# yuki-koyama/sequential-line-search

Measured on AMD Instinct MI355X. Metric: GP-fit+acq-max step time (ms) and candidate-evals/sec at N=8192 D=64, higher is better.
Workload: dtype f64

## Files before the change

sequential-line-search_amd/csrc/capi.hip:

```cpp
#include <cstddef>
#include <cstring>
#include <algorithm>
#include <cmath>
#include <cstdlib>
#include <cstring>
#include <atomic>
#include <map>
#include <memory>
#include <condition_variable>
#include <mutex>
#include <shared_mutex>

#include "common.hpp"
#include "kernels.hpp"
#include "lbfgs_driver.hpp"

using namespace slsk;


namespace slsk {
static thread_local char g_err[512] = "";
void set_error(const char* fmt, ...) {
    va_list ap;
    va_start(ap, fmt);
// ... 303 lines not shown
    if (!ctx) return SLS_ERR_INVALID;
    CtxCall call_(ctx);
    (void)hipStreamSynchronize(ctx->stream);
    ctx->prof_collect();
    ctx->prof.clear();
    return SLS_OK;
}
extern "C" int sls_prof_get(sls_ctx* ctx, const char* name, double* total_ms, long* launches) {
    if (!ctx || !name) return SLS_ERR_INVALID;
    CtxCall call_(ctx);
    (void)hipStreamSynchronize(ctx->stream);
    ctx->prof_collect();
    if (std::string(name) == "potrf_fallbacks") {
        if (total_ms) *total_ms = 0.0;
        if (launches) *launches = ctx->potrf_fallbacks;
        return SLS_OK;
    }
    auto it = ctx->prof.find(name);
    if (total_ms) *total_ms = it == ctx->prof.end() ? 0.0 : it->second.ms;
    if (launches) *launches = it == ctx->prof.end() ? 0 : it->second.launches;
    return SLS_OK;
}

static void h2d(sls_ctx* c, double* dst, const double* src, size_t n) {
    SLS_HIP(hipMemcpyAsync(dst, src, n * sizeof(double), hipMemcpyHostToDevice, c->stream));
}
static void d2h(sls_ctx* c, double* dst, const double* src, size_t n) {
    SLS_HIP(hipMemcpyAsync(dst, src, n * sizeof(double), hipMemcpyDeviceToHost, c->stream));
}
static void sync(sls_ctx* c) { SLS_HIP(hipStreamSynchronize(c->stream)); }
static const size_t IO_STAGE_MAX = (size_t)4 << 20;

static void check_theta(const double* theta, int D) {
    SLS_REQUIRE(theta != nullptr, "theta is NULL");
    SLS_REQUIRE(theta[0] > 0.0, "theta[0] (signal variance) must be positive");
    for (int d = 0; d < D; ++d) SLS_REQUIRE(theta[1 + d] > 0.0, "length scale %d must be positive", d);
}

static void d2h_matrix(sls_ctx* c, double* dst, const double* src, int N, int Np) {
    SLS_HIP(hipMemcpy2DAsync(dst, (size_t)N * 8, src, (size_t)Np * 8, (size_t)N * 8, N, hipMemcpyDeviceToHost, c->stream));
}
static void h2d_matrix(sls_ctx* c, double* dst, const double* src, int N, int Np) {
    SLS_HIP(hipMemcpy2DAsync(dst, (size_t)Np * 8, src, (size_t)N * 8, (size_t)N * 8, N, hipMemcpyHostToDevice, c->stream));
}

struct sls_gp {
    sls_ctx* ctx = nullptr;
    int D = 0, N = 0, Np = 0, Dp = 0, Dcols = 0, kernel = 0;
    double a = 0, b = 0;
    std::vector<double> theta, Xh, yh;
    std::vector<double> il_h, ypad_h;
    bool host_stale = false;
    DBuf X, y, inv_ell, XT, XaT, nx, L, Linv, Kinv, U, alpha, tvec, mu_data, scal, gemv_part, idx_buf;
    const double* linv_clean_p = nullptr;
    int linv_clean_np = 0;
    long* d_idx = nullptr;
    HostBuf sum;
    int best_index = 0;
    double mu_best = 0, logdet = 0;
    DBuf Ks, Cs, P, Vs, parts, Gs, Gm, Gpart, XsT, ns, raw, outv;
    int ws_chunk = 0;
    DBuf pair_mu, pair_sg, pair_dmu, pair_dsg;
    LbfgsWs lb;
    DBuf eubo_Ks, eubo_Cs, eubo_XsT, eubo_ns, eubo_parts, eubo_Gs, eubo_Gm, eubo_Kd;
    int eubo_chunk = 0, eubo_np = 0;
    HostBuf eubo_best;
    int sigma_mode = 0;
    long generation = 0;
    long stat_issued = 0, stat_cap = 0;
    int stat_rounds = 0, stat_live_end = 0;
    HostBuf zc;
    HostBuf io;
    double* io_stage(size_t doubles) {
        if (io.host && doubles * 8 > io.bytes) (void)hipStreamSynchronize(ctx->stream);
        io.ensure(ctx, doubles * 8, false);
        return io.host;
    }
    std::shared_mutex state_mtx;
};

static bool gp_fit_small_ok(const sls_gp* g) {
    if (g->N > NLL_SMALL_MAX_N || g->Np != 128 || g->D > 128) return false;
    return tune_on(TUNE_FIT_SMALL);
}

static std::atomic<long> g_gp_generation{0};
static void gp_fit_device(sls_gp* g) {
    g->generation = ++g_gp_generation;
    sls_ctx* c = g->ctx;
    const int N = g->N, Np = g->Np, D = g->D;
    if (gp_fit_small_ok(g)) {
        GpFitSmallArgs f;
        f.X = g->X.p; f.y = g->y.p; f.inv_ell = g->inv_ell.p;
        f.D = D; f.N = N; f.Dcols = g->Dcols; f.a = g->a; f.b = g->b;
        f.XT = g->XT.p; f.nx = g->nx.p; f.XaT = g->XaT.p; f.L = g->L.p; f.Linv = g->Linv.p; f.U = g->U.p; f.Kinv = g->Kinv.p;
        f.alpha = g->alpha.p; f.mu_data = g->mu_data.p; f.scal = g->scal.p; f.d_idx = g->d_idx; f.info = c->d_info;
        f.summary = g->sum.dev;
        f.x_lds = tune_on(TUNE_SMALL_XLDS) ? 1 : 0;
        SLS_HIP(hipMemsetAsync(c->d_info, 0, 64, c->stream));
        ProfScope ps(c, "fit_small");
        launch_gp_fit_small(c->stream, g->kernel, f);
        return;
    }
    KernelSpec ks{g->kernel, g->a};
    {
        ProfScope ps(c, "gram");
        launch_prep_points(c->stream, g->X.p, D, N, g->inv_ell.p, g->XT.p, Np, Np, g->Dcols, g->nx.p);
        launch_gram_sym(c->stream, g->XT.p, Np, g->Dp, g->nx.p, Np, N, ks, g->b, g->L.p, true);
    }
    SLS_HIP(hipMemsetAsync(c->d_info, 0, 64, c->stream));
    if (g->linv_clean_p != g->Linv.p || g->linv_clean_np != Np) {
        launch_fill(c->stream, g->Linv.p, (long)Np * Np, 0.0);
        g->linv_clean_p = g->Linv.p;
        g->linv_clean_np = Np;
    }
    c->potrf_tick_rearm();
    int* df_sync = c->potrf_df_sync(Np);
    if (potri_fused_applies(Np, df_sync != nullptr)) {
        ProfScope ps(c, "potri");
        if (!launch_potri(c->stream, g->L.p, Np, g->Linv.p, g->U.p, g->Kinv.p, c->d_info, df_sync))
            ps.rename("potrf+trtri+lauum");
    } else {
        {
            ProfScope ps(c, "potrf");
            launch_potrf(c->stream, g->L.p, Np, g->Linv.p, c->d_info, 0, df_sync);
        }
        {
            ProfScope ps(c, "trtri");
            launch_trtri(c->stream, g->L.p, Np, g->Linv.p, g->Kinv.p, g->U.p);
        }
        {
            ProfScope ps(c, "lauum");
            launch_lauum(c->stream, g->U.p, Np, g->Kinv.p);
        }
    }
    launch_gemv_n(c->stream, g->Linv.p, Np, g->y.p, g->tvec.p, g->gemv_part.p, true);
    launch_gemv_t(c->stream, g->Linv.p, Np, g->tvec.p, g->alpha.p, true);
    launch_scale_rows(c->stream, g->XT.p, g->alpha.p, g->XaT.p, Np, Np, g->Dcols);
    if (g->sigma_mode == 1) launch_transpose_full(c->stream, g->Linv.p, g->U.p, Np);
    launch_fit_summary(c->stream, g->y.p, g->alpha.p, g->b, N, g->mu_data.p, g->L.p, Np, c->d_info, g->scal.p, g->d_idx, g->sum.dev);
}

static void gp_fetch_summary(sls_gp* g, int attempt = 0) {
    sls_ctx* c = g->ctx;
    sync(c);
    const double* sm = g->sum.host;
    const int info[2] = {(int)sm[3], (int)sm[4]};
    if (potrf_gave_up(c, info[1], attempt)) {
        gp_fit_device(g);
        gp_fetch_summary(g, 1);
        return;
    }
    if (info[0] != 0) {
        set_error("Cholesky failed: K_y is not positive definite (pivot %d)", info[0] - 1);
        throw HipFail{SLS_ERR_NOT_SPD};
    }
    g->best_index = (int)sm[2];
    g->mu_best = sm[0];
    g->logdet = sm[1];
}
static void gp_setup(sls_gp* g) {
    sls_ctx* ctx = g->ctx;
    const int D = g->D, N = (int)g->yh.size();
    g->N = N;
    g->Np = round_up(N, 128); g->Dp = round_up(D, 16); g->Dcols = round_up(D, 128);
    const size_t Np = g->Np;
    g->X.ensure((size_t)D * N); g->y.ensure(Np); g->inv_ell.ensure(g->Dcols);
    g->XT.ensure(Np * g->Dcols); g->XaT.ensure(Np * g->Dcols); g->nx.ensure(Np);
    g->L.ensure(Np * Np); g->Linv.ensure(Np * Np); g->Kinv.ensure(Np * Np); g->U.ensure(Np * Np);
    g->alpha.ensure(Np); g->tvec.ensure(Np); g->mu_data.ensure(Np); g->scal.ensure(8);
    g->gemv_part.ensure((Np / 128) * Np);
    g->ws_chunk = 0;
    g->idx_buf.ensure(8);
    g->d_idx = reinterpret_cast<long*>(g->idx_buf.p);
    g->sum.ensure(ctx, (size_t)(16 + D) * 8, true);
    g->il_h.assign(g->Dcols, 0.0);
    g->ypad_h.assign(Np, 0.0);
    for (int d = 0; d < D; ++d) g->il_h[d] = 1.0 / g->theta[1 + d];
    std::copy(g->yh.begin(), g->yh.end(), g->ypad_h.begin());
    h2d(ctx, g->X.p, g->Xh.data(), (size_t)D * N);
    h2d(ctx, g->y.p, g->ypad_h.data(), Np);
    h2d(ctx, g->inv_ell.p, g->il_h.data(), g->Dcols);
    gp_fit_device(g);
    gp_fetch_summary(g);
}

extern "C" int sls_gp_create(sls_ctx* ctx, const double* X, int D, int N, const double* y, const double* theta, double b,
                             int kernel, sls_gp** out) {
    SLS_TRY
    CtxCall call_(ctx);
    SLS_REQUIRE(ctx && out, "sls_gp_create: NULL argument");
// ... 181 lines not shown
    return tune_on(TUNE_TRI_PREDICT);
}

static void eval_candidates(sls_gp* g, const double* xr, long ldr, int S, const EvalOut& o, bool point_major = false) {
    sls_ctx* c = g->ctx;
    const int Np = g->Np, N = g->N, D = g->D;
    const bool want_grad = o.dmu || o.dsigma || o.grad;
    const int chunk_max = std::min(round_up(S, 128), c->cand_chunk);
    ensure_eval_ws(g, chunk_max);
    const int nbt = Np / 128;
    KernelSpec ks{g->kernel, g->a};
    for (int s0 = 0; s0 < S; s0 += chunk_max) {
        const int sc = std::min(chunk_max, S - s0);
        const int Sp = round_up(sc, 128);
        const long ldk = Sp;
        double* Cs = (g->kernel == SLS_KERNEL_ARD_MATERN52) ? g->Cs.p : g->Ks.p;
        double* mu_part = g->parts.p;
        double* ca_part = mu_part + (size_t)nbt * ldk;
        double* kw_part = ca_part + (size_t)nbt * ldk;
        double* cw_part = kw_part + (size_t)2 * nbt * ldk;
        {
            ProfScope ps(c, "cross_gram");
            if (point_major) launch_prep_points(c->stream, xr + (size_t)s0 * D, D, sc, g->inv_ell.p, g->XsT.p, ldk, Sp, g->Dcols, g->ns.p);
            else launch_prep_cands(c->stream, xr + s0, ldr, D, sc, g->inv_ell.p, g->XsT.p, ldk, Sp, g->Dcols, g->ns.p);
            launch_cross_gram(c->stream, g->XsT.p, ldk, g->ns.p, Sp, g->XT.p, Np, g->nx.p, Np, N, g->Dp, ks, g->alpha.p, g->Ks.p, Cs,
                              ldk, mu_part, ca_part);
        }
        int split_first = 0x7fffffff;
        const bool solve_grad = g->sigma_mode == 1 && (want_grad || !tri_predict());
        {
            ProfScope ps(c, want_grad ? "acq_gemm" : "var_gemm");
            if (solve_grad) {
                g->Vs.ensure((size_t)chunk_max * Np);
                launch_gemm_plain(c->stream, g->Ks.p, ldk, false, g->Linv.p, Np, false, g->Vs.p, ldk, Sp / 128, Np / 128, Np, 1.0, 0.0);
                split_first = launch_acq_gemm(c->stream, g->Vs.p, Cs, ldk, Sp, g->U.p, Np, g->P.p, kw_part, cw_part, c->d_info + 32);
            } else if (want_grad || !tri_predict())
                split_first = launch_acq_gemm(c->stream, g->Ks.p, Cs, ldk, Sp, g->Kinv.p, Np, g->P.p, kw_part, cw_part, c->d_info + 32);
            else
                launch_var_gemm(c->stream, g->Ks.p, ldk, Sp, g->Linv.p, Np, kw_part, cw_part);
        }
        double* kw_solve = nullptr;
        if (solve_grad) {
            kw_solve = cw_part + (size_t)2 * nbt * ldk;
            ProfScope ps(c, "var_gemm");
            launch_var_gemm(c->stream, g->Ks.p, ldk, Sp, g->Linv.p, Np, kw_solve, kw_solve + (size_t)2 * nbt * ldk);
        }
        if (want_grad) {
            ProfScope ps(c, "grad_gemm");
            double* part = nullptr;
            if (D <= 64 && grad_gemm_wants_split(Sp)) {
                g->Gpart.ensure((size_t)8 * Sp * 64);
                part = g->Gpart.p;
            }
            launch_grad_gemm(c->stream, g->P.p, Cs, ldk, Sp, g->XT.p, g->XaT.p, Np, Np, D <= 64 ? -g->Dcols : g->Dcols, g->Gs.p, g->Gm.p,
                             part);
        }
        {
            ProfScope ps(c, "finalize");
            FinalizeArgs f;
            f.S = sc; f.D = D; f.nbt = nbt; f.ldk = ldk; f.ntm = Sp / 128; f.split_first = split_first;
            f.mu_part = mu_part; f.ca_part = ca_part; f.kw_part = kw_part; f.cw_part = cw_part;
            f.kw_solve_part = kw_solve;
            f.Gs = g->Gs.p; f.Gm = g->Gm.p; f.XsT = g->XsT.p; f.inv_ell = g->inv_ell.p;
            f.a = g->a; f.mu_best = g->mu_best; f.ucb_h = o.ucb_h; f.acq = o.acq;
            f.ldo = o.ldo;
            f.mu = o.mu ? o.mu + s0 : nullptr;
            f.sigma = o.sigma ? o.sigma + s0 : nullptr;
            f.dmu = o.dmu ? o.dmu + s0 : nullptr;
            f.dsigma = o.dsigma ? o.dsigma + s0 : nullptr;
            f.val = o.val ? o.val + s0 : nullptr;
            f.grad = o.grad ? o.grad + s0 : nullptr;
            launch_finalize(c->stream, f);
        }
    }
}

constexpr int WAVE_PATH_MAX_POINTS = 4096;
static bool wave_path_dims(const sls_gp* g) { return tune_on(TUNE_WAVE_PATH) && g->D <= WAVE_PATH_MAX_D; }
static bool wave_path_applies(const sls_gp* g, int count) {
    return wave_path_dims(g) && g->Np <= WAVE_PATH_MAX_NP && count <= WAVE_PATH_MAX_POINTS;
}
static void wave_model_args(const sls_gp* g, WaveArgs& w) {
    w.D = g->D; w.N = g->N; w.Np = g->Np;
    w.matern = g->kernel == SLS_KERNEL_ARD_MATERN52;
    w.a = g->a; w.mu_best = g->mu_best;
    w.XT = g->XT.p; w.inv_ell = g->inv_ell.p; w.Kinv = g->Kinv.p; w.alpha = g->alpha.p;
    w.solve_sigma = g->sigma_mode == 1; w.Linv = g->Linv.p; w.U = g->U.p;
    w.useful = nullptr;
}
static void wave_eval(const sls_gp* g, hipStream_t s, const double* Xs_dev, int M, const EvalOut& o) {
    WaveArgs w;
    wave_model_args(g, w);
    w.S = M; w.m = 1; w.n_local = 0; w.acq = o.acq; w.ucb_h = o.ucb_h;
    w.c1 = 0; w.shrink = 0; w.gtol = 0; w.max_backtracks = 0;
    w.starts = Xs_dev; w.x_out = nullptr; w.f_out = nullptr; w.ld = o.ldo;
    w.ev_mu = o.mu; w.ev_sigma = o.sigma; w.ev_dmu = o.dmu; w.ev_dsigma = o.dsigma; w.ev_val = o.val; w.ev_grad = o.grad;
    launch_maximize_wave(s, w);
}
static void eval_small(sls_gp* g, const double* Xs_dev, int M, const EvalOut& o) {
    ProfScope ps(g->ctx, "acq_wave");
    wave_eval(g, g->ctx->stream, Xs_dev, M, o);
}

static void upload_candidates(sls_gp* g, const double* Xs, int M, DBuf& raw, int Mp) {
    sls_ctx* c = g->ctx;
    const int D = g->D;
    std::vector<double> t((size_t)Mp * D, 0.5);
    for (int m = 0; m < M; ++m)
// ... 538 lines not shown
    const bool matern = g->kernel == SLS_KERNEL_ARD_MATERN52;
    const bool solve = g->sigma_mode == 1;
    if (solve) g->Vs.ensure((size_t)chunk_max * Np);
    KernelSpec ks{g->kernel, g->a};
    for (int s0 = 0; s0 < S; s0 += chunk_max) {
        const int sc = std::min(chunk_max, S - s0);
        const int Sp = round_up(sc, 128);
        const long ldk = Sp;
        double* Ks[2] = {g->Ks.p, g->eubo_Ks.p};
        double* Cs[2] = {matern ? g->Cs.p : g->Ks.p, matern ? g->eubo_Cs.p : g->eubo_Ks.p};
        double* XsT[2] = {g->XsT.p, g->eubo_XsT.p};
        double* ns[2] = {g->ns.p, g->eubo_ns.p};
        double* Gs[2] = {g->Gs.p, g->eubo_Gs.p};
        double* Gm[2] = {g->Gm.p, g->eubo_Gm.p};
        double* mu_part[2] = {g->parts.p, g->eubo_parts.p};
        double *ca_part[2], *kw_part[2], *cw_part[2];
        for (int o = 0; o < 2; ++o) {
            ca_part[o] = mu_part[o] + (size_t)nbt * ldk;
            kw_part[o] = ca_part[o] + (size_t)nbt * ldk;
            cw_part[o] = kw_part[o] + (size_t)2 * nbt * ldk;
        }
        double* kw_solve = solve ? cw_part[0] + (size_t)2 * nbt * ldk : nullptr;
        for (int o = 0; o < 2; ++o) {
            ProfScope ps(c, "cross_gram");
            launch_prep_cands(c->stream, xr + (size_t)o * D * ldr + s0, ldr, D, sc, g->inv_ell.p, XsT[o], ldk, Sp, g->Dcols, ns[o]);
            launch_cross_gram(c->stream, XsT[o], ldk, ns[o], Sp, g->XT.p, Np, g->nx.p, Np, N, g->Dp, ks, g->alpha.p, Ks[o], Cs[o], ldk,
                              mu_part[o], ca_part[o]);
        }
        {
            ProfScope ps(c, "eubo");
            launch_pair_diff(c->stream, Ks[0], Ks[1], ldk, Np, g->eubo_Kd.p);
        }
        if (solve) {
            {
                ProfScope ps(c, "acq_gemm");
                launch_gemm_plain(c->stream, g->eubo_Kd.p, ldk, false, g->Linv.p, Np, false, g->Vs.p, ldk, Sp / 128, Np / 128, Np, 1.0, 0.0);
            }
            ProfScope ps(c, "var_gemm");
            launch_var_gemm(c->stream, g->eubo_Kd.p, ldk, Sp, g->Linv.p, Np, kw_solve, kw_solve + (size_t)2 * nbt * ldk);
        }
        int split_first = 0x7fffffff;
        for (int o = 0; o < 2; ++o) {
            {
                ProfScope ps(c, "acq_gemm");
                split_first = launch_acq_gemm(c->stream, solve ? g->Vs.p : g->eubo_Kd.p, Cs[o], ldk, Sp, solve ? g->U.p : g->Kinv.p, Np,
                                              g->P.p, kw_part[o], cw_part[o], c->d_info + 32);
            }
            ProfScope ps(c, "grad_gemm");
            double* part = nullptr;
            if (D <= 64 && grad_gemm_wants_split(Sp)) {
                g->Gpart.ensure((size_t)8 * Sp * 64);
                part = g->Gpart.p;
            }
            launch_grad_gemm(c->stream, g->P.p, Cs[o], ldk, Sp, g->XT.p, g->XaT.p, Np, Np, D <= 64 ? -g->Dcols : g->Dcols, Gs[o], Gm[o], part);
        }
        {
            ProfScope ps(c, "eubo");
            EuboFinalizeArgs f;
            f.S = sc; f.D = D; f.nbt = nbt; f.ntm = Sp / 128; f.split_first = split_first; f.kernel = g->kernel; f.ldk = ldk;
            for (int o = 0; o < 2; ++o) {
                f.mu_part[o] = mu_part[o]; f.ca_part[o] = ca_part[o]; f.cw_part[o] = cw_part[o];
                f.Gs[o] = Gs[o]; f.Gm[o] = Gm[o]; f.XsT[o] = XsT[o];
            }
            f.kw_part = kw_part[0]; f.kw_solve_part = kw_solve; f.inv_ell = g->inv_ell.p; f.a = g->a;
            f.ldo = ldo;
            f.val = val ? val + s0 : nullptr;
            f.grad = grad ? grad + s0 : nullptr;
            launch_eubo_finalize(c->stream, f);
        }
    }
}

extern "C" int sls_eubo_eval(sls_gp* g, const double* pairs, int M, double* val, double* grad) {
    SLS_TRY
    CtxCall call_(g);
    SLS_REQUIRE(g != nullptr, "sls_eubo_eval: gp is NULL");
    SLS_REQUIRE(pairs != nullptr, "sls_eubo_eval: pairs is NULL");
    SLS_REQUIRE(M >= 0, "sls_eubo_eval: M = %d", M);
    if (M == 0) return SLS_OK;
    std::shared_lock<std::shared_mutex> state_(g->state_mtx);
    sls_ctx* c = g->ctx;
    const int Mp = round_up(M, 128), D2 = 2 * g->D;
    std::vector<double> t((size_t)Mp * D2, 0.5);
    for (int m = 0; m < M; ++m)
        for (int r = 0; r < D2; ++r) t[(size_t)m + (size_t)r * Mp] = pairs[r + (size_t)m * D2];
    g->raw.ensure((size_t)Mp * D2);
    h2d(c, g->raw.p, t.data(), (size_t)Mp * D2);
    sync(c);
    std::vector<double> unused;
    if (!val) unused.resize(M);
    EvalOut want;
    want.val = val ? val : unused.data(); want.grad = grad;
    const size_t n = eval_block_doubles(want, D2, Mp);
    g->outv.ensure(n);
    const EvalOut o = eval_block(want, g->outv.p, D2, Mp);
    eval_pairs(g, g->raw.p, Mp, M, o.val, o.grad, Mp);
    std::vector<double> pageable;
    eval_block_to_host(want, eval_block(want, fetch(g, g->outv.p, n, pageable), D2, Mp), D2, M);
    SLS_CATCH
}

extern "C" int sls_eubo_maximize(sls_gp* g, const double* starts, int S, int n_local, const sls_lbfgs_opts* opts,
                                 long start_index_offset, double* x_out, double* val_out, long* idx_out, double* x_stars,
                                 double* y_stars) {
    SLS_TRY
    CtxCall call_(g);
    SLS_REQUIRE(g != nullptr, "sls_eubo_maximize: gp is NULL");
// ... 161 lines not shown
    launch_diag_inverse(c->stream, Ld.p, Np, Li.p);
    launch_trtri(c->stream, Ld.p, Np, Li.p, Ki.p, Ui.p);
    launch_lauum(c->stream, Ui.p, Np, Ki.p);
    d2h_matrix(c, Ainv, Ki.p, N, Np);
    sync(c);
    SLS_CATCH
}

extern "C" int sls_gp_append_point(sls_gp* g, const double* x, double y_new) {
    SLS_TRY
    CtxCall call_(g);
    SLS_REQUIRE(g && x, "sls_gp_append_point: NULL argument");
    std::unique_lock<std::shared_mutex> state_(g->state_mtx);
    sls_ctx* c = g->ctx;
    const int D = g->D, N = g->N, Np = g->Np;
    if (g->host_stale) {
        d2h(c, g->Xh.data(), g->X.p, (size_t)D * N);
        d2h(c, g->yh.data(), g->y.p, (size_t)N);
        sync(c);
        g->host_stale = false;
    }
    g->Xh.insert(g->Xh.end(), x, x + D);
    g->yh.push_back(y_new);
    if (N % 128 == 0) {
        gp_setup(g);
        return SLS_OK;
    }
    upload_candidates(g, x, 1, g->raw, 128);
    ensure_eval_ws(g, 128);
    g->outv.ensure(4 * (size_t)Np + 8);
    double* kvec = g->outv.p;
    double* uvec = kvec + Np;
    double* lvec = uvec + Np;
    double* tmp = lvec + Np;
    double* scal = tmp + Np;
    KernelSpec ks{g->kernel, g->a};
    launch_prep_cands(c->stream, g->raw.p, 128, D, 1, g->inv_ell.p, g->XsT.p, 128, 128, g->Dcols, g->ns.p);
    double* Cs = (g->kernel == SLS_KERNEL_ARD_MATERN52) ? g->Cs.p : g->Ks.p;
    launch_cross_gram(c->stream, g->XsT.p, 128, g->ns.p, 128, g->XT.p, Np, g->nx.p, Np, N, g->Dp, ks, nullptr, g->Ks.p, Cs, 128,
                      nullptr, nullptr);
    SLS_HIP(hipMemcpy2DAsync(kvec, 8, g->Ks.p, 128 * 8, 8, Np, hipMemcpyDeviceToDevice, c->stream));
    launch_gemv_n(c->stream, g->Kinv.p, Np, kvec, uvec, g->gemv_part.p);
    launch_gemv_n(c->stream, g->Linv.p, Np, kvec, lvec, g->gemv_part.p, true);
    launch_append_dots(c->stream, kvec, uvec, lvec, g->y.p, N, scal);
    const double kappa = g->a + g->b;
    launch_append_update(c->stream, g->Kinv.p, g->L.p, g->Linv.p, g->alpha.p, Np, N, uvec, lvec, scal, kappa, y_new);
    SLS_HIP(hipMemcpyAsync(g->y.p + N, &g->yh[N], 8, hipMemcpyHostToDevice, c->stream));
    g->X.ensure((size_t)D * (N + 1));
    SLS_HIP(hipMemcpyAsync(g->X.p, g->Xh.data(), (size_t)D * (N + 1) * 8, hipMemcpyHostToDevice, c->stream));
    g->N = N + 1;
    g->generation = ++g_gp_generation;
    launch_prep_points(c->stream, g->X.p, D, N + 1, g->inv_ell.p, g->XT.p, Np, Np, g->Dcols, g->nx.p);
    launch_scale_rows(c->stream, g->XT.p, g->alpha.p, g->XaT.p, Np, Np, g->Dcols);
    if (g->sigma_mode == 1) launch_transpose_full(c->stream, g->Linv.p, g->U.p, Np);
    SLS_HIP(hipMemsetAsync(c->d_info, 0, 64, c->stream));
    launch_fit_summary(c->stream, g->y.p, g->alpha.p, g->b, N + 1, g->mu_data.p, g->L.p, Np, c->d_info, g->scal.p, g->d_idx, g->sum.dev);
    gp_fetch_summary(g);
    SLS_REQUIRE(std::isfinite(g->logdet), "sls_gp_append_point: the extended K_y is not positive definite");
    SLS_CATCH
}
```

sequential-line-search_amd/csrc/gemm_f64.hpp:

```cpp
#pragma once
#include <hip/hip_runtime.h>

namespace slsk {

typedef double d4_t __attribute__((ext_vector_type(4)));
typedef double d2_t __attribute__((ext_vector_type(2)));

constexpr int GEMM_BM = 128;
constexpr int GEMM_BN = 128;
constexpr int GEMM_BK = 16;
constexpr int GEMM_THREADS = 256;
constexpr int GEMM_LDS_MC_LD = 144;
constexpr int GEMM_LDS_KC_LD = 18;
constexpr int GEMM_LDS_TILE = 16 * 144;
constexpr int GEMM_LDS_BYTES = 4 * GEMM_LDS_TILE * 8;

struct Acc {
    d4_t v[4][4];
    __device__ __forceinline__ void zero() {
#pragma unroll
        for (int i = 0; i < 4; ++i)
#pragma unroll
            for (int j = 0; j < 4; ++j) v[i][j] = d4_t{0.0, 0.0, 0.0, 0.0};
    }
// ... 260 lines not shown
    };
    constexpr bool DIRECT_A = !A_KC;
    const int wave_u = __builtin_amdgcn_readfirstlane(tid >> 6);
    auto issue_a = [&](int k0, int bufoff) {
#pragma unroll
        for (int r = 0; r < 4; ++r) {
            const int row = 4 * wave_u + r;
            slab_row_to_lds(A + 2 * lane + (long)(k0 + row) * lda, lds + bufoff + row * A_LD);
        }
    };
    if (DIRECT_A) issue_a(kb, 0);
    else stage_load<A_KC>(sa, A, lda, kb, tid);
    load_b(kb);
    if (DIRECT_A) asm volatile("s_waitcnt vmcnt(0)" ::: "memory");
    else stage_store<A_KC>(sa, lds, tid);
    store_b(lds + A_SLAB);
    __syncthreads();
    int cur = 0;
    for (int k0 = kb; k0 < ke; k0 += GEMM_BK) {
        const bool more = (k0 + GEMM_BK) < ke;
        if (more) {
            if (DIRECT_A) issue_a(k0 + GEMM_BK, cur ^ BUF);
            else stage_load<A_KC>(sa, A, lda, k0 + GEMM_BK, tid);
            load_b(k0 + GEMM_BK);
        }
        const double* la = lds + cur;
        const double* lb = lds + cur + A_SLAB;
#pragma unroll
        for (int kk = 0; kk < 4; ++kk) {
            double af[2], bf[4];
#pragma unroll
            for (int i = 0; i < 2; ++i)
                af[i] = A_KC ? frag_read<true>(la, wm + 16 * i, kk, lane)
                             : la[(4 * kk + (lane >> 4)) * A_LD + wm + 16 * i + (lane & 15)];
#pragma unroll
            for (int j = 0; j < 4; ++j) bf[j] = frag_read<true>(lb, 16 * j, kk, lane);
#pragma unroll
            for (int i = 0; i < 2; ++i)
#pragma unroll
                for (int j = 0; j < 4; ++j)
                    acc.v[i][j] = __builtin_amdgcn_mfma_f64_16x16x4f64(bf[j], af[i], acc.v[i][j], 0, 0, 0);
        }
        const int nxt = cur ^ BUF;
        if (more) {
            if (!DIRECT_A) stage_store<A_KC>(sa, lds + nxt, tid);
            store_b(lds + nxt + A_SLAB);
        }
        if (DIRECT_A) asm volatile("s_waitcnt vmcnt(0)" ::: "memory");
        __syncthreads();
        cur = nxt;
    }
}

__device__ __forceinline__ int acc_m(int i) {
    const int lane = threadIdx.x & 63, wave = threadIdx.x >> 6;
    return (wave & 1) * 64 + 16 * i + (lane & 15);
}
__device__ __forceinline__ int acc_n(int j, int r) {
    const int lane = threadIdx.x & 63, wave = threadIdx.x >> 6;
    return (wave >> 1) * 64 + 16 * j + (lane >> 4) + 4 * r;
}

template <bool HEAVY = false, class F>
__device__ __forceinline__ void acc_tile_by_columns(const Acc& acc, double* lds, F&& f) {
    const int lane = threadIdx.x & 63, wave = __builtin_amdgcn_readfirstlane(threadIdx.x >> 6);
#pragma unroll
    for (int half = 0; half < 2; ++half) {
        __syncthreads();
        if ((wave >> 1) == half) {
#pragma unroll
            for (int i = 0; i < 4; ++i)
#pragma unroll
                for (int j = 0; j < 4; ++j)
#pragma unroll
                    for (int r = 0; r < 4; ++r)
                        lds[(16 * j + (lane >> 4) + 4 * r) * GEMM_LDS_MC_LD + (wave & 1) * 64 + 16 * i + (lane & 15)] = acc.v[i][j][r];
        }
        __syncthreads();
        if constexpr (HEAVY) {
#pragma unroll 2
            for (int q = 0; q < 16; ++q) {
                const int c = wave + 4 * q;
                const d2_t v = *reinterpret_cast<const d2_t*>(lds + c * GEMM_LDS_MC_LD + 2 * lane);
                f(64 * half + c, 2 * lane, v);
            }
        } else {
#pragma unroll
            for (int q = 0; q < 16; ++q) {
                const int c = wave + 4 * q;
                const d2_t v = *reinterpret_cast<const d2_t*>(lds + c * GEMM_LDS_MC_LD + 2 * lane);
                f(64 * half + c, 2 * lane, v);
            }
        }
    }
}

__device__ __forceinline__ int xcd_remap(int b, int nwg) {
    const int q = nwg >> 3, r = nwg & 7;
    const int xcd = b & 7, within = b >> 3;
    const int base = (xcd < r) ? xcd * (q + 1) : r * (q + 1) + (xcd - r) * q;
    return base + within;
}

}
```

sequential-line-search_amd/csrc/kernels.hpp:

```cpp
#pragma once
#include <cstdlib>
#include <hip/hip_runtime.h>

#include "tuning.hpp"
#include "../../include/sls_hip.h"

#include <mutex>
#include <map>
#include <set>
#include <utility>

namespace slsk {

inline void ensure_dyn_lds(const void* fn, int bytes) {
    static std::mutex mtx;
    static std::map<std::pair<int, const void*>, int> done;
    int dev = 0;
    (void)hipGetDevice(&dev);
    std::lock_guard<std::mutex> lock(mtx);
    int& have = done[{dev, fn}];
    if (bytes > have) {
        if (hipFuncSetAttribute(fn, hipFuncAttributeMaxDynamicSharedMemorySize, bytes) != hipSuccess) (void)hipGetLastError();
        have = bytes;
    }
// ... 69 lines not shown
};
void launch_nll_small(hipStream_t s, int kernel, const NllSmallArgs& args);

struct GpFitSmallArgs {
    const double *X, *y, *inv_ell;
    int D, N, Dcols;
    double a, b;
    double *XT, *nx, *XaT, *L, *Linv, *U, *Kinv, *alpha, *mu_data, *scal;
    long* d_idx;
    int* info;
    double* summary = nullptr;
    int x_lds = 1;
};
void launch_gp_fit_small(hipStream_t s, int kernel, const GpFitSmallArgs& args);

constexpr int MAP_OPT_MAX_VARS = 320;
constexpr int MAP_OPT_HIST = 8;
constexpr int MAP_OPT_TRACE_SLOTS = 24;
constexpr int MAP_OPT_STATE_DOUBLES = (4 + 2 * MAP_OPT_HIST) * MAP_OPT_MAX_VARS + 32;
constexpr int MAP_OPT_OUT_X = 8, MAP_OPT_OUT_G = 8 + MAP_OPT_MAX_VARS, MAP_OPT_OUT_DOUBLES = 8 + 2 * MAP_OPT_MAX_VARS;
struct MapOptArgs {
    const double* X;
    const double* XTr;
    double* kc;
    int x_lds = 1;
    int D, N, ny, nh, log_hyper, noiseless;
    const double* y_fixed;
    double a0, b0, r0;
    double mu_a, mu_b, mu_r, s2_a, s2_b, s2_r;
    double btl_scale;
    int n_prefs, flat_len;
    const int *pref_off, *pref_flat;
    const int *csc_off, *csc_ent;
    double* btl_scratch;
    const double *z0, *lower, *upper;
    int max_evals;
    double ftol_rel, xtol_rel;
    int budget;
    int eval_only;
    int fresh;
    double* state;
    double* out;
    int* info;
    long long* trace;
};
void launch_map_opt(hipStream_t s, int kernel, const MapOptArgs& args);

int launch_acq_gemm(hipStream_t s, const double* Ks, const double* Cs, long ldk, int Sp, const double* Kinv, int Np, double* P,
                    double* kw_part, double* cw_part, int* sync = nullptr);
void launch_var_gemm(hipStream_t s, const double* Ks, long ldk, int Sp, const double* Linv, int Np, double* kw_part,
                     double* cw_part);
inline bool grad_gemm_wants_split(int Sp) { return !tune_set(TUNE_GRAD_SPLIT_TILES) || 2 * (Sp / 128) < tune(TUNE_GRAD_SPLIT_TILES, 0); }
void launch_grad_gemm(hipStream_t s, const double* P, const double* Cs, long ldk, int Sp, const double* XT, const double* XaT,
                      long ld, int Np, int Dcols, double* Gs, double* Gm, double* part = nullptr, int passes = 2);
struct FinalizeArgs {
    int S, D, nbt;
    int ntm, split_first;
    long ldk;
    const double *mu_part, *ca_part, *kw_part, *cw_part, *Gs, *Gm, *XsT, *inv_ell;
    const double* kw_solve_part = nullptr;
    double a, mu_best, ucb_h;
    int acq;
    long ldo;
    double *mu, *sigma, *dmu, *dsigma, *val, *grad;
};
void launch_finalize(hipStream_t s, const FinalizeArgs& a);

void launch_combine(hipStream_t s, int S, int D, long ld, const double* mu, const double* sigma, const double* dmu,
                    const double* dsigma, int acq, double mu_best, double ucb_h, double* val, double* grad);

void launch_mes_combine(hipStream_t s, int S, int D, long ld, const double* mu, const double* sigma, const double* dmu,
                        const double* dsigma, const double* y_star, int K, double* val, double* grad);
void launch_mes_terms(hipStream_t s, const double* t, long n, double* g, double* dg);

void launch_logei_combine(hipStream_t s, int S, int D, long ld, const double* mu, const double* sigma, const double* dmu,
                          const double* dsigma, double mu_best, double* val, double* grad);
void launch_logei_terms(hipStream_t s, const double* u, long n, double* log_h, double* b1, double* b2);

void launch_pair_diff(hipStream_t s, const double* Ka, const double* Kb, long ldk, int Np, double* Kd);
struct EuboFinalizeArgs {
    int S, D, nbt;
    int ntm, split_first;
    int kernel;
    long ldk;
    const double *mu_part[2], *ca_part[2], *cw_part[2], *Gs[2], *Gm[2], *XsT[2];
    const double *kw_part, *inv_ell;
    const double* kw_solve_part = nullptr;
    double a;
    long ldo;
    double *val, *grad;
};
void launch_eubo_finalize(hipStream_t s, const EuboFinalizeArgs& a);

struct LbfgsState {
    int S, D, m;
    long ld;
    double *x, *g, *dir, *xt, *scr;
    double *Sh, *Yh;
    double *rho;
    double *f, *t;
    int *hlen, *hpos, *nbt, *done;
    double c1, shrink, gtol;
    int max_backtracks;
    double ftol_rel = 0.0, xtol_rel = 0.0;
    const int* live;
    int nlive;
    long ldv;
// ... 121 lines not shown
```

sequential-line-search_amd/csrc/kernels_acq.hip:

```cpp
#include <cstdlib>

#include "gemm_f64.hpp"
#include "kernels.hpp"
#include "../../include/sls_hip.h"

namespace slsk {

template <bool MATERN, bool HALF>
__device__ __forceinline__ void acq_tile(int t, int nhalf, int ntm, int ntn, const double* __restrict__ Ks, const double* __restrict__ Cs,
                                         long ldk, const double* __restrict__ Kinv, int Np, double* __restrict__ P,
                                         double* __restrict__ kw_part, double* __restrict__ cw_part, double* lds) {
    const int GM = 8;
    const int gsz = GM * ntn;
    const int g = t / gsz, w = t % gsz;
    const int gm = min(GM, ntm - g * GM);
    const int tm = g * GM + (w % gm), tn = w / gm;
    const int m0 = tm * GEMM_BM, n0 = tn * GEMM_BN;
    Acc acc;
    acc.zero();
    gemm_tile<false, false, HALF ? 2 : 4, true>(acc, Ks + m0, ldk, Kinv + n0, (long)Np, 0, Np, lds, nhalf);
    const int lane = threadIdx.x & 63, wave = threadIdx.x >> 6;
    constexpr int NJ = HALF ? 2 : 4;
    const int nbase = HALF ? 64 * nhalf + (wave >> 1) * 32 : (wave >> 1) * 64;
    double* red = lds;
// ... 253 lines not shown
    const int ntm = Sp / GEMM_BM;
    const int tm = blockIdx.x % ntm, tn = blockIdx.x / ntm;
    const int m0 = tm * GEMM_BM, n0 = tn * GEMM_BN;
    const double* A = blockIdx.y == 0 ? P : Cs;
    const double* B = blockIdx.y == 0 ? XT : XaT;
    double* C = blockIdx.y == 0 ? Gs : Gm;
    Acc acc;
    acc.zero();
    gemm_tile<false, true>(acc, A + m0, ldk, B + (long)n0 * ld, ld, 0, Np, lds);
#pragma unroll
    for (int i = 0; i < 4; ++i)
#pragma unroll
        for (int j = 0; j < 4; ++j)
#pragma unroll
            for (int r = 0; r < 4; ++r) C[(long)(m0 + acc_m(i)) + (long)(n0 + acc_n(j, r)) * ldk] = acc.v[i][j][r];
}

constexpr int GRAD64_A_LD = 136;
__global__ __launch_bounds__(256, 3) void grad_gemm64_kernel(const double* __restrict__ P, const double* __restrict__ Cs, long ldk,
                                                             int Sp, const double* __restrict__ XT, const double* __restrict__ XaT,
                                                             long ld, int Np, double* __restrict__ Gs, double* __restrict__ Gm,
                                                             double* __restrict__ part) {
    extern __shared__ __attribute__((aligned(16))) char smem[];
    double* lds = reinterpret_cast<double*>(smem);
    const int m0 = blockIdx.x * GEMM_BM;
    const double* A = blockIdx.y == 0 ? P : Cs;
    const double* B = blockIdx.y == 0 ? XT : XaT;
    const bool split = gridDim.z > 1;
    double* C = split ? part + ((long)blockIdx.z * 2 + blockIdx.y) * (long)Sp * 64 : (blockIdx.y == 0 ? Gs : Gm);
    const long ldc = split ? (long)Sp : ldk;
    const int q = Np / 4;
    Acc64 tot;
    tot.zero();
    const int c0 = split ? blockIdx.z : 0, c1 = split ? blockIdx.z + 1 : 4;
    for (int c = c0; c < c1; ++c) {
        Acc64 acc;
        acc.zero();
        gemm_tile_n64<false, GRAD64_A_LD>(acc, A + m0, ldk, B, ld, c * q, (c + 1) * q, lds);
#pragma unroll
        for (int i = 0; i < 2; ++i)
#pragma unroll
            for (int j = 0; j < 4; ++j) tot.v[i][j] = (c == c0) ? acc.v[i][j] : tot.v[i][j] + acc.v[i][j];
    }
    const int lane = threadIdx.x & 63, wm = (threadIdx.x >> 6) * 32;
#pragma unroll
    for (int i = 0; i < 2; ++i)
#pragma unroll
        for (int j = 0; j < 4; ++j)
#pragma unroll
            for (int r = 0; r < 4; ++r)
                C[(long)(m0 + wm + 16 * i + (lane & 15)) + (long)(16 * j + (lane >> 4) + 4 * r) * ldc] = tot.v[i][j][r];
}

__global__ __launch_bounds__(256) void grad_reduce4_kernel(const double* __restrict__ part, int Sp, long ldk, double* __restrict__ Gs,
                                                           double* __restrict__ Gm, int passes) {
    const long idx = blockIdx.x * 256L + threadIdx.x;
    if (idx >= (long)Sp * 64) return;
    const long n = idx % Sp, d = idx / Sp;
    const long stride = (long)Sp * 64;
    for (int y = 0; y < passes; ++y) {
        const double* p = part + (long)y * stride + idx;
        const double v = ((p[0] + p[2 * stride]) + p[4 * stride]) + p[6 * stride];
        (y == 0 ? Gs : Gm)[n + d * ldk] = v;
    }
}

void launch_grad_gemm(hipStream_t s, const double* P, const double* Cs, long ldk, int Sp, const double* XT, const double* XaT,
                      long ld, int Np, int Dcols, double* Gs, double* Gm, double* part, int passes) {
    ensure_dyn_lds((const void*)grad_gemm_kernel, GEMM_LDS_BYTES);
    ensure_dyn_lds((const void*)grad_gemm64_kernel, gemm_n64_lds_bytes<GRAD64_A_LD>());
    if (Dcols < 0) {
        const bool split = part != nullptr && grad_gemm_wants_split(Sp);
        hipLaunchKernelGGL(grad_gemm64_kernel, dim3(Sp / GEMM_BM, passes, split ? 4 : 1), dim3(GEMM_THREADS), gemm_n64_lds_bytes<GRAD64_A_LD>(), s, P, Cs,
                           ldk, Sp, XT, XaT, ld, Np, Gs, Gm, part);
        if (split)
            hipLaunchKernelGGL(grad_reduce4_kernel, dim3((unsigned)(((long)Sp * 64 + 255) / 256)), dim3(256), 0, s, part, Sp, ldk, Gs, Gm,
                               passes);
        return;
    }
    const int nt = (Sp / GEMM_BM) * (Dcols / GEMM_BN);
    hipLaunchKernelGGL(grad_gemm_kernel, dim3(nt, passes), dim3(GEMM_THREADS), GEMM_LDS_BYTES, s, P, Cs, ldk, Sp, XT, XaT, ld, Np, Dcols,
                       Gs, Gm);
}

__global__ __launch_bounds__(256) void finalize_kernel(FinalizeArgs p) {
    const int n = blockIdx.x * 256 + threadIdx.x;
    if (n >= p.S) return;
    double mu = 0.0, ca = 0.0, kw = 0.0, cw = 0.0;
    const int tm_ = n >> 7, grp_ = tm_ >> 3;
    const int gm_ = min(8, p.ntm - 8 * grp_);
    const int tile_base = grp_ * 8 * p.nbt + (tm_ - 8 * grp_);
    #pragma unroll 8
    for (int t = 0; t < p.nbt; ++t) {
        mu += p.mu_part[(long)t * p.ldk + n];
        ca += p.ca_part[(long)t * p.ldk + n];
        double kt = p.kw_part[(long)(2 * t) * p.ldk + n], ct = p.cw_part[(long)(2 * t) * p.ldk + n];
        if (tile_base + t * gm_ >= p.split_first) {
            kt += p.kw_part[(long)(2 * t + 1) * p.ldk + n];
            ct += p.cw_part[(long)(2 * t + 1) * p.ldk + n];
        }
        kw += kt;
        cw += ct;
    }
    if (p.kw_solve_part) {
        kw = 0.0;
        for (int t = 0; t < p.nbt; ++t) kw += p.kw_solve_part[(long)(2 * t) * p.ldk + n];
    }
    const double s2 = p.a - kw;
    const double sigma = s2 < 0.0 ? 0.0 : sqrt(s2);
    if (p.mu) p.mu[n] = mu;
    if (p.sigma) p.sigma[n] = sigma;
    const bool need_g = p.dmu || p.dsigma || p.grad;
    double Phi = 0.0, phi = 0.0;
    bool bad = false;
    if (p.val || p.grad) {
        if (p.acq == SLS_ACQ_EXPECTED_IMPROVEMENT) {
            const double diff = mu - p.mu_best;
            const double u = diff / sigma;
            Phi = 0.5 * erfc(-u * 0.70710678118654752440);
            phi = exp(-0.5 * u * u) * 0.39894228040143267794;
            const double ei = diff * Phi + sigma * phi;
            bad = (sigma < 1e-10) || isnan(ei);
            if (p.val) p.val[n] = bad ? 0.0 : ei;
        } else {
            if (p.val) p.val[n] = mu + p.ucb_h * sigma;
        }
    }
// ... 689 lines not shown
```

sequential-line-search_amd/csrc/tuning.hpp:

```cpp
#pragma once
#include <atomic>
#include <cstdlib>
#include <mutex>

namespace slsk {
#define SLS_TUNING_KEYS(X)                                                                                                      \
    X(POOL_MB) X(FIT_SMALL) X(TRI_PREDICT) X(WAVE_PATH) X(IO_STAGE) X(EVAL_ZEROCOPY) X(WAVE_TRACE) X(COMPACT) \
    X(NLL_SMALL) X(SMALL_ZEROCOPY) X(NLL_BATCH) X(MAP_DEVICE) X(MAP_TRACE) X(SMALL_XLDS) X(MULTI_RCCL) X(PERSIST)                \
    X(ACQ_WG_PER_CU) X(GATE_PHASE) X(TAIL_SPLIT) X(LBFGS_REG) X(TRI_WG_PER_CU) X(POTRF_MODE) X(POTRF_DNBO) X(POTRF_NBO)          \
    X(LAUUM_N64) X(TRTRI_NARROW) X(POTRI_FUSED) X(POTRF_STREAM) X(POTRF_SPLIT) X(POTRI_W1) X(POTRF_TIMEOUT_TICKS) X(POTRF_DNEAR) X(POTRI_PLAST)  \
    X(POTRI_CX) X(POTRI_CK) X(WAVE_STAGE) X(WAVE_COOP) X(GRAD_SPLIT_TILES) X(EVAL_SLOTS) X(GATE_EVERY) X(POTRF_FUSE_SYRK) X(POTRI_POOL) X(POTRF_POOL) X(POTRI_POOL_KEEP) X(POTRI_POOL_NEAR) X(POTRI_POOL_NEAR_W)
enum TuneKey {
#define SLS_TK(name) TUNE_##name,
    SLS_TUNING_KEYS(SLS_TK)
#undef SLS_TK
    TUNE_COUNT
};
struct SlsTuning {
    std::atomic<long long> word[TUNE_COUNT];
};
namespace tuning_detail {
inline SlsTuning& table() {
    static SlsTuning t;
    return t;
}
inline void parse() {
    static const char* const names[TUNE_COUNT] = {
#define SLS_TK(name) "SLS_" #name,
        SLS_TUNING_KEYS(SLS_TK)
#undef SLS_TK
    };
    SlsTuning& t = table();
    for (int k = 0; k < TUNE_COUNT; ++k) {
        const char* v = getenv(names[k]);
        t.word[k].store(v ? (((long long)atol(v)) << 1) | 1 : 0, std::memory_order_relaxed);
    }
}
}
inline const SlsTuning& tuning() {
    static std::once_flag once;
    std::call_once(once, tuning_detail::parse);
    return tuning_detail::table();
}
inline void tuning_reload() {
    (void)tuning();
    tuning_detail::parse();
}
inline long tune(TuneKey k, long dflt) {
    const long long w = tuning().word[k].load(std::memory_order_relaxed);
    return (w & 1) ? (long)(w >> 1) : dflt;
}
inline bool tune_on(TuneKey k, bool dflt = true) { return tune(k, dflt ? 1 : 0) != 0; }
inline bool tune_set(TuneKey k) { return (tuning().word[k].load(std::memory_order_relaxed) & 1) != 0; }

}
```

Baseline: 535,000.

## Use point-major copies of X and X*alpha for the D<=64 gradient GEMM

After each fit, the code now builds point-major (row = point, 64 contiguous dims) copies of XT and XaT with a small LDS transpose kernel. A new grad_gemm64d kernel then reads the B operand as contiguous 64-wide rows into double-buffered LDS, with swizzled reads feeding f64 MFMA. The goal is cheaper, coalesced B-tile loads in the acquisition gradient GEMM. The cost is an extra transpose per fit and two extra Np×64 buffers, and a generation check rebuilds the copies when they are stale.

```diff
diff --git a/sequential-line-search_amd/csrc/capi.hip b/sequential-line-search_amd/csrc/capi.hip
--- a/sequential-line-search_amd/csrc/capi.hip
+++ b/sequential-line-search_amd/csrc/capi.hip
@@ -379,6 +379,8 @@
     std::vector<double> il_h, ypad_h;
     bool host_stale = false;
     DBuf X, y, inv_ell, XT, XaT, nx, L, Linv, Kinv, U, alpha, tvec, mu_data, scal, gemv_part, idx_buf;
+    DBuf XD, XaD;
+    long xd_generation = -1;
     const double* linv_clean_p = nullptr;
     int linv_clean_np = 0;
     long* d_idx = nullptr;
@@ -412,6 +414,18 @@
 }
 
 static std::atomic<long> g_gp_generation{0};
+static bool gp_dmajor_wanted(const sls_gp* g) { return g->D <= 64 && tune(TUNE_GRAD_B_LAYOUT, 1) != 0; }
+static void gp_build_dmajor(sls_gp* g) {
+    g->XD.ensure((size_t)g->Np * 64);
+    g->XaD.ensure((size_t)g->Np * 64);
+    launch_dmajor_copy(g->ctx->stream, g->XT.p, g->XaT.p, g->Np, g->Np, g->XD.p, g->XaD.p);
+    g->xd_generation = g->generation;
+}
+static bool gp_grad_dmajor(sls_gp* g) {
+    if (!gp_dmajor_wanted(g)) return false;
+    if (g->xd_generation != g->generation) gp_build_dmajor(g);
+    return true;
+}
 static void gp_fit_device(sls_gp* g) {
     g->generation = ++g_gp_generation;
     sls_ctx* c = g->ctx;
@@ -464,6 +478,7 @@
     launch_gemv_n(c->stream, g->Linv.p, Np, g->y.p, g->tvec.p, g->gemv_part.p, true);
     launch_gemv_t(c->stream, g->Linv.p, Np, g->tvec.p, g->alpha.p, true);
     launch_scale_rows(c->stream, g->XT.p, g->alpha.p, g->XaT.p, Np, Np, g->Dcols);
+    if (gp_dmajor_wanted(g)) gp_build_dmajor(g);
     if (g->sigma_mode == 1) launch_transpose_full(c->stream, g->Linv.p, g->U.p, Np);
     launch_fit_summary(c->stream, g->y.p, g->alpha.p, g->b, N, g->mu_data.p, g->L.p, Np, c->d_info, g->scal.p, g->d_idx, g->sum.dev);
 }
@@ -751,8 +766,9 @@
                 g->Gpart.ensure((size_t)8 * Sp * 64);
                 part = g->Gpart.p;
             }
+            const bool dmaj = gp_grad_dmajor(g);
             launch_grad_gemm(c->stream, g->P.p, Cs, ldk, Sp, g->XT.p, g->XaT.p, Np, Np, D <= 64 ? -g->Dcols : g->Dcols, g->Gs.p, g->Gm.p,
-                             part);
+                             part, 2, dmaj ? g->XD.p : nullptr, dmaj ? g->XaD.p : nullptr);
         }
         {
             ProfScope ps(c, "finalize");
@@ -1397,7 +1413,9 @@
                 g->Gpart.ensure((size_t)8 * Sp * 64);
                 part = g->Gpart.p;
             }
-            launch_grad_gemm(c->stream, g->P.p, Cs[o], ldk, Sp, g->XT.p, g->XaT.p, Np, Np, D <= 64 ? -g->Dcols : g->Dcols, Gs[o], Gm[o], part);
+            const bool dmaj = gp_grad_dmajor(g);
+            launch_grad_gemm(c->stream, g->P.p, Cs[o], ldk, Sp, g->XT.p, g->XaT.p, Np, Np, D <= 64 ? -g->Dcols : g->Dcols, Gs[o], Gm[o], part,
+                             2, dmaj ? g->XD.p : nullptr, dmaj ? g->XaD.p : nullptr);
         }
         {
             ProfScope ps(c, "eubo");
@@ -1665,6 +1683,7 @@
     g->generation = ++g_gp_generation;
     launch_prep_points(c->stream, g->X.p, D, N + 1, g->inv_ell.p, g->XT.p, Np, Np, g->Dcols, g->nx.p);
     launch_scale_rows(c->stream, g->XT.p, g->alpha.p, g->XaT.p, Np, Np, g->Dcols);
+    if (gp_dmajor_wanted(g)) gp_build_dmajor(g);
     if (g->sigma_mode == 1) launch_transpose_full(c->stream, g->Linv.p, g->U.p, Np);
     SLS_HIP(hipMemsetAsync(c->d_info, 0, 64, c->stream));
     launch_fit_summary(c->stream, g->y.p, g->alpha.p, g->b, N + 1, g->mu_data.p, g->L.p, Np, c->d_info, g->scal.p, g->d_idx, g->sum.dev);
diff --git a/sequential-line-search_amd/csrc/gemm_f64.hpp b/sequential-line-search_amd/csrc/gemm_f64.hpp
--- a/sequential-line-search_amd/csrc/gemm_f64.hpp
+++ b/sequential-line-search_amd/csrc/gemm_f64.hpp
@@ -336,6 +336,68 @@
     }
 }
 
+constexpr int GEMM_N64D_LDS_A = 16 * 128, GEMM_N64D_LDS_B = 16 * 64;
+constexpr int GEMM_N64D_LDS_BUF = GEMM_N64D_LDS_A + GEMM_N64D_LDS_B;
+constexpr int GEMM_N64D_LDS_BYTES = 2 * GEMM_N64D_LDS_BUF * 8;
+__device__ __forceinline__ void gemm_tile_n64d(Acc64& acc, const double* __restrict__ A, long lda, const double* __restrict__ Bd,
+                                               int kb, int ke, double* lds) {
+    if (kb >= ke) return;
+    const int tid = threadIdx.x, lane = tid & 63;
+    const int wave = __builtin_amdgcn_readfirstlane(tid >> 6);
+    const int wm = wave * 32;
+    const unsigned lds_base = (unsigned)(unsigned long long)(__attribute__((address_space(3))) double*)lds;
+    const unsigned a_even = 16u * lane, a_odd = (16u * lane) ^ 128u;
+    const unsigned b_off = 8u * ((lane >> 5) * 64 + (((2 * lane) & 63) ^ (16 * (lane >> 5))));
+    const double* Arow = A + (long)(kb + 4 * wave) * lda;
+    const double* Brow = Bd + (long)(kb + 4 * wave) * 64;
+    auto issue = [&](int bufoff) {
+#pragma unroll
+        for (int r = 0; r < 4; ++r)
+            slab_row_to_lds_saddr(Arow + (long)r * lda, (r & 1) ? a_odd : a_even, lds_base + 8u * (unsigned)(bufoff + (4 * wave + r) * 128));
+#pragma unroll
+        for (int t = 0; t < 2; ++t)
+            slab_row_to_lds_saddr(Brow + 128 * t, b_off, lds_base + 8u * (unsigned)(bufoff + GEMM_N64D_LDS_A + (4 * wave + 2 * t) * 64));
+    };
+    const int sw = 16 * ((lane >> 4) & 1);
+    int a_rd[2], b_rd[4];
+#pragma unroll
+    for (int i = 0; i < 2; ++i) a_rd[i] = (lane >> 4) * 128 + (((wm + (lane & 15)) ^ sw) ^ (16 * i));
+#pragma unroll
+    for (int j = 0; j < 4; ++j) b_rd[j] = (lane >> 4) * 64 + (((lane & 15) ^ sw) ^ (16 * j));
+    auto compute = [&](int bufoff) {
+        const double* la = lds + bufoff;
+        const double* lb = lds + bufoff + GEMM_N64D_LDS_A;
+#pragma unroll
+        for (int kk = 0; kk < 4; ++kk) {
+            double af[2], bf[4];
+#pragma unroll
+            for (int i = 0; i < 2; ++i) af[i] = la[4 * kk * 128 + a_rd[i]];
+#pragma unroll
+            for (int j = 0; j < 4; ++j) bf[j] = lb[4 * kk * 64 + b_rd[j]];
+#pragma unroll
+            for (int i = 0; i < 2; ++i)
+#pragma unroll
+                for (int j = 0; j < 4; ++j)
+                    acc.v[i][j] = __builtin_amdgcn_mfma_f64_16x16x4f64(bf[j], af[i], acc.v[i][j], 0, 0, 0);
+        }
+    };
+    issue(0);
+    ring_wait_barrier<0>();
+    const int nslab = (ke - kb) / GEMM_BK;
+    for (int s = 0; s < nslab; s += 2) {
+        Arow += (long)GEMM_BK * lda;
+        Brow += GEMM_BK * 64;
+        issue(GEMM_N64D_LDS_BUF);
+        compute(0);
+        ring_wait_barrier<0>();
+        Arow += (long)GEMM_BK * lda;
+        Brow += GEMM_BK * 64;
+        if (s + 2 < nslab) issue(0);
+        compute(GEMM_N64D_LDS_BUF);
+        ring_wait_barrier<0>();
+    }
+}
+
 __device__ __forceinline__ int acc_m(int i) {
     const int lane = threadIdx.x & 63, wave = threadIdx.x >> 6;
     return (wave & 1) * 64 + 16 * i + (lane & 15);
diff --git a/sequential-line-search_amd/csrc/kernels.hpp b/sequential-line-search_amd/csrc/kernels.hpp
--- a/sequential-line-search_amd/csrc/kernels.hpp
+++ b/sequential-line-search_amd/csrc/kernels.hpp
@@ -145,7 +145,9 @@
                      double* cw_part);
 inline bool grad_gemm_wants_split(int Sp) { return !tune_set(TUNE_GRAD_SPLIT_TILES) || 2 * (Sp / 128) < tune(TUNE_GRAD_SPLIT_TILES, 0); }
 void launch_grad_gemm(hipStream_t s, const double* P, const double* Cs, long ldk, int Sp, const double* XT, const double* XaT,
-                      long ld, int Np, int Dcols, double* Gs, double* Gm, double* part = nullptr, int passes = 2);
+                      long ld, int Np, int Dcols, double* Gs, double* Gm, double* part = nullptr, int passes = 2,
+                      const double* XD = nullptr, const double* XaD = nullptr);
+void launch_dmajor_copy(hipStream_t s, const double* XT, const double* XaT, long ld, int Np, double* XD, double* XaD);
 struct FinalizeArgs {
     int S, D, nbt;
     int ntm, split_first;
diff --git a/sequential-line-search_amd/csrc/kernels_acq.hip b/sequential-line-search_amd/csrc/kernels_acq.hip
--- a/sequential-line-search_amd/csrc/kernels_acq.hip
+++ b/sequential-line-search_amd/csrc/kernels_acq.hip
@@ -329,6 +329,63 @@
                 C[(long)(m0 + wm + 16 * i + (lane & 15)) + (long)(16 * j + (lane >> 4) + 4 * r) * ldc] = tot.v[i][j][r];
 }
 
+__global__ __launch_bounds__(256, 3) void grad_gemm64d_kernel(const double* __restrict__ P, const double* __restrict__ Cs, long ldk,
+                                                              int Sp, const double* __restrict__ XD, const double* __restrict__ XaD,
+                                                              int Np, double* __restrict__ Gs, double* __restrict__ Gm,
+                                                              double* __restrict__ part) {
+    extern __shared__ __attribute__((aligned(16))) char smem[];
+    double* lds = reinterpret_cast<double*>(smem);
+    const int m0 = blockIdx.x * GEMM_BM;
+    const double* A = blockIdx.y == 0 ? P : Cs;
+    const double* B = blockIdx.y == 0 ? XD : XaD;
+    const bool split = gridDim.z > 1;
+    double* C = split ? part + ((long)blockIdx.z * 2 + blockIdx.y) * (long)Sp * 64 : (blockIdx.y == 0 ? Gs : Gm);
+    const long ldc = split ? (long)Sp : ldk;
+    const int q = Np / 4;
+    Acc64 tot;
+    tot.zero();
+    const int c0 = split ? blockIdx.z : 0, c1 = split ? blockIdx.z + 1 : 4;
+    for (int c = c0; c < c1; ++c) {
+        Acc64 acc;
+        acc.zero();
+        gemm_tile_n64d(acc, A + m0, ldk, B, c * q, (c + 1) * q, lds);
+#pragma unroll
+        for (int i = 0; i < 2; ++i)
+#pragma unroll
+            for (int j = 0; j < 4; ++j) tot.v[i][j] = (c == c0) ? acc.v[i][j] : tot.v[i][j] + acc.v[i][j];
+    }
+    const int lane = threadIdx.x & 63, wm = (threadIdx.x >> 6) * 32;
+#pragma unroll
+    for (int i = 0; i < 2; ++i)
+#pragma unroll
+        for (int j = 0; j < 4; ++j)
+#pragma unroll
+            for (int r = 0; r < 4; ++r)
+                C[(long)(m0 + wm + 16 * i + (lane & 15)) + (long)(16 * j + (lane >> 4) + 4 * r) * ldc] = tot.v[i][j][r];
+}
+
+__global__ __launch_bounds__(256) void dmajor_copy_kernel(const double* __restrict__ XT, const double* __restrict__ XaT, long ld,
+                                                          double* __restrict__ XD, double* __restrict__ XaD) {
+    __shared__ double t[64 * 65];
+    const int i0 = blockIdx.x * 64, l = threadIdx.x & 63, w = threadIdx.x >> 6;
+    const double* src = blockIdx.y == 0 ? XT : XaT;
+    double* dst = blockIdx.y == 0 ? XD : XaD;
+#pragma unroll
+    for (int k = 0; k < 16; ++k) {
+        const int d = w + 4 * k;
+        t[l * 65 + d] = src[(long)(i0 + l) + (long)d * ld];
+    }
+    __syncthreads();
+#pragma unroll
+    for (int k = 0; k < 16; ++k) {
+        const int i = w + 4 * k;
+        dst[(long)(i0 + i) * 64 + l] = t[i * 65 + l];
+    }
+}
+void launch_dmajor_copy(hipStream_t s, const double* XT, const double* XaT, long ld, int Np, double* XD, double* XaD) {
+    hipLaunchKernelGGL(dmajor_copy_kernel, dim3(Np / 64, 2), dim3(256), 0, s, XT, XaT, ld, XD, XaD);
+}
+
 __global__ __launch_bounds__(256) void grad_reduce4_kernel(const double* __restrict__ part, int Sp, long ldk, double* __restrict__ Gs,
                                                            double* __restrict__ Gm, int passes) {
     const long idx = blockIdx.x * 256L + threadIdx.x;
@@ -343,13 +400,19 @@
 }
 
 void launch_grad_gemm(hipStream_t s, const double* P, const double* Cs, long ldk, int Sp, const double* XT, const double* XaT,
-                      long ld, int Np, int Dcols, double* Gs, double* Gm, double* part, int passes) {
+                      long ld, int Np, int Dcols, double* Gs, double* Gm, double* part, int passes, const double* XD,
+                      const double* XaD) {
     ensure_dyn_lds((const void*)grad_gemm_kernel, GEMM_LDS_BYTES);
     ensure_dyn_lds((const void*)grad_gemm64_kernel, gemm_n64_lds_bytes<GRAD64_A_LD>());
+    ensure_dyn_lds((const void*)grad_gemm64d_kernel, GEMM_N64D_LDS_BYTES);
     if (Dcols < 0) {
         const bool split = part != nullptr && grad_gemm_wants_split(Sp);
-        hipLaunchKernelGGL(grad_gemm64_kernel, dim3(Sp / GEMM_BM, passes, split ? 4 : 1), dim3(GEMM_THREADS), gemm_n64_lds_bytes<GRAD64_A_LD>(), s, P, Cs,
-                           ldk, Sp, XT, XaT, ld, Np, Gs, Gm, part);
+        if (XD != nullptr && (passes < 2 || XaD != nullptr))
+            hipLaunchKernelGGL(grad_gemm64d_kernel, dim3(Sp / GEMM_BM, passes, split ? 4 : 1), dim3(GEMM_THREADS), GEMM_N64D_LDS_BYTES, s, P,
+                               Cs, ldk, Sp, XD, XaD, Np, Gs, Gm, part);
+        else
+            hipLaunchKernelGGL(grad_gemm64_kernel, dim3(Sp / GEMM_BM, passes, split ? 4 : 1), dim3(GEMM_THREADS),
+                               gemm_n64_lds_bytes<GRAD64_A_LD>(), s, P, Cs, ldk, Sp, XT, XaT, ld, Np, Gs, Gm, part);
         if (split)
             hipLaunchKernelGGL(grad_reduce4_kernel, dim3((unsigned)(((long)Sp * 64 + 255) / 256)), dim3(256), 0, s, part, Sp, ldk, Gs, Gm,
                                passes);
diff --git a/sequential-line-search_amd/csrc/tuning.hpp b/sequential-line-search_amd/csrc/tuning.hpp
--- a/sequential-line-search_amd/csrc/tuning.hpp
+++ b/sequential-line-search_amd/csrc/tuning.hpp
@@ -9,7 +9,8 @@
     X(NLL_SMALL) X(SMALL_ZEROCOPY) X(NLL_BATCH) X(MAP_DEVICE) X(MAP_TRACE) X(SMALL_XLDS) X(MULTI_RCCL) X(PERSIST)                \
     X(ACQ_WG_PER_CU) X(GATE_PHASE) X(TAIL_SPLIT) X(LBFGS_REG) X(TRI_WG_PER_CU) X(POTRF_MODE) X(POTRF_DNBO) X(POTRF_NBO)          \
     X(LAUUM_N64) X(TRTRI_NARROW) X(POTRI_FUSED) X(POTRF_STREAM) X(POTRF_SPLIT) X(POTRI_W1) X(POTRF_TIMEOUT_TICKS) X(POTRF_DNEAR) X(POTRI_PLAST)  \
-    X(POTRI_CX) X(POTRI_CK) X(WAVE_STAGE) X(WAVE_COOP) X(GRAD_SPLIT_TILES) X(EVAL_SLOTS) X(GATE_EVERY) X(POTRF_FUSE_SYRK) X(POTRI_POOL) X(POTRF_POOL) X(POTRI_POOL_KEEP) X(POTRI_POOL_NEAR) X(POTRI_POOL_NEAR_W)
+    X(POTRI_CX) X(POTRI_CK) X(WAVE_STAGE) X(WAVE_COOP) X(GRAD_SPLIT_TILES) X(EVAL_SLOTS) X(GATE_EVERY) X(POTRF_FUSE_SYRK) X(POTRI_POOL) X(POTRF_POOL) X(POTRI_POOL_KEEP) X(POTRI_POOL_NEAR) X(POTRI_POOL_NEAR_W) \
+    X(GRAD_B_LAYOUT)
 enum TuneKey {
 #define SLS_TK(name) TUNE_##name,
     SLS_TUNING_KEYS(SLS_TK)
```

Measured after the change: 535,100 (median of 3 runs). No clear change (+0.0%).
